# BenChung/SuccessiveConvexification

Measured on AMD Instinct MI355X. Metric: 6-DoF K=50 SCvx iterations/sec (batch), higher is better.
Workload: dtype f64

## Files before the change

successiveconvexification_amd/csrc/scvx_ipm_core.hpp:

```cpp
#pragma once
#include <math.h>
#include <stdint.h>
#include <type_traits>

#if defined(__HIPCC__)
#define SCVX_HD __host__ __device__ __forceinline__
#define SCVX_HD_NI __host__ __device__ __attribute__((noinline))
#else
#define SCVX_HD inline
#define SCVX_HD_NI inline
#endif
#if defined(SCVX_IPM_PROF) && defined(__HIP_DEVICE_COMPILE__)
#define SCVX_TS(v) const unsigned long long v = __builtin_amdgcn_s_memtime()
#define SCVX_TE(v, slot) prof[slot] += (double)(__builtin_amdgcn_s_memtime() - v)
#else
#define SCVX_TS(v)
#define SCVX_TE(v, slot)
#endif
#ifndef SCVX_NODE_QR
#define SCVX_NODE_QR 0
#endif
#ifndef SCVX_STALL_ITERS
#define SCVX_STALL_ITERS 3
#endif
#ifndef SCVX_INIT_BALANCE
#define SCVX_INIT_BALANCE 1.0
#endif
#ifndef SCVX_INIT_SHIFT
#define SCVX_INIT_SHIFT 0.25
#endif
#ifndef SCVX_WARM_RADIUS
#define SCVX_WARM_RADIUS 0.999
#endif
#ifndef SCVX_BLEND_WARM
#define SCVX_BLEND_WARM 0.0
#endif
#ifndef SCVX_BLEND_RADIUS
#define SCVX_BLEND_RADIUS 0.9
#endif
#ifndef SCVX_STEP_FRAC
#define SCVX_STEP_FRAC 0.98
#endif
#ifndef SCVX_REFINE_PRED
#define SCVX_REFINE_PRED 0
#endif
#ifndef SCVX_BLOWUP_STOP
#define SCVX_BLOWUP_STOP 10.0
#endif
#ifndef SCVX_WARM_SAVE
#define SCVX_WARM_SAVE 1.0
#endif
#ifndef SCVX_FACTOR_T
#define SCVX_FACTOR_T double
#endif
#ifndef SCVX_STREAM_U
#define SCVX_STREAM_U 4
#endif
#ifndef SCVX_REFINE_FROM
#define SCVX_REFINE_FROM 1e-4
#endif
#ifndef SCVX_REFINE_FUSED
#define SCVX_REFINE_FUSED 1
#endif
#ifndef SCVX_FUSED_RES
#define SCVX_FUSED_RES 0
#endif
#ifndef SCVX_NEWTON_CORR_ATTR
#define SCVX_NEWTON_CORR_ATTR SCVX_HD
#endif
#ifndef SCVX_CARRY_BIGSUMS
#define SCVX_CARRY_BIGSUMS 0
#endif
#ifndef SCVX_RESID_UPDATE
#define SCVX_RESID_UPDATE 1
#endif
#ifndef SCVX_RESID_FRESH_FROM
#define SCVX_RESID_FRESH_FROM 1e-4
#endif
#ifndef SCVX_TWISTED_TSPACE
#define SCVX_TWISTED_TSPACE 1
#endif
#ifndef SCVX_REFINE_STOP
#define SCVX_REFINE_STOP 0.1
#endif
#if defined(__HIPCC__)
#define SCVX_UNROLL _Pragma("unroll")
#else
#define SCVX_UNROLL
#endif
#if defined(__HIP_DEVICE_COMPILE__) && !defined(SCVX_NO_LDS_FRAME)
#define SCVX_THIS_LDS() do { __builtin_assume(__builtin_amdgcn_is_shared((const void*)this)); __builtin_assume(__builtin_amdgcn_is_shared((const void*)&C)); } while (0)
#else
#define SCVX_THIS_LDS() do { } while (0)
#endif
#define SCVX_T0() SCVX_TS(t0_)
#define SCVX_T1(slot) SCVX_TE(t0_, slot)
#if defined(SCVX_IPM_DEBUG) && !defined(__HIPCC__)
#include <stdio.h>
#ifndef SCVX_DBG_NODE
#define SCVX_DBG_NODE -1
#endif
#define SCVX_DBG(...) fprintf(stderr, __VA_ARGS__)
#else
#define SCVX_DBG(...)
#endif

#if defined(SCVX_COUNTERS) && !defined(__HIPCC__)
extern "C" long long scvx_counters[8];
#define SCVX_COUNT(i) do { _Pragma("omp atomic") scvx_counters[i]++; } while (0)
#else
#define SCVX_COUNT(i)
#endif

namespace scvx {
namespace ipm {

#if defined(__HIP_DEVICE_COMPILE__)
#define SCVX_GLOBAL __attribute__((address_space(1)))
#else
#define SCVX_GLOBAL
#endif
template <class T> struct gp {
    typedef SCVX_GLOBAL T elem;
    typedef elem* ptr;
    typedef const elem* cptr;
};
typedef gp<double>::elem gdouble;
typedef gp<double>::ptr gptr;
typedef gp<double>::cptr cgptr;

struct Consts {
    int K, max_iter, refine, pad;
    int warm, retries;
    double tol, accept;
    double itan, sqcm, icos, Tmax, Tmin, omMax, mdry, wNu, mwet;
    double finmxf;
    double vmax;
    double rIf[3], vIf[3], qBIf[4], wBi[3], wBf[3];
};

enum { LINV_SZ = 105 };
SCVX_HD int linv_row(int i) { return i < 7 ? 15 * i : 15 * (13 - i) + (14 - i); }

enum { HX_M = 0, HX_R = 1, HX_V = 10, HX_Q = 19, HX_Q34 = 20, HX_W = 24, HX_SZ = 33 };
SCVX_HD constexpr int hu_size(int nu) { return nu == 5 ? 13 : 9; }

struct Layout {
    int K, nx, nu_, nloc, nv, iS, iTNU, iTTR, iTS;
    int o_gs, o_tilt, o_rate, o_mass, o_tb, o_tc, o_lb, o_fin, o_dp, o_nu, o_tr, o_sg, o_rk, nc;
    int c_gs, c_tilt, c_rate, c_mass, c_tb, c_tc, c_lb, c_fin, c_dp, c_nu, c_tr, c_sg, c_rk, ncones, nsmall;
    int ndp, nfin, NU;
    int ny;
    SCVX_HD void init(int K_, bool with_dp = false, int nu = 3) {
        K = K_;
        NU = nu == 5 ? 5 : 3;
        ndp = with_dp ? K_ : 0;
        nfin = NU == 5 ? K_ + 1 : 0;
        nx = 14 * (K + 1);
        nu_ = NU * (K + 1);
        nloc = nx + nu_ + 14 * K;
        iS = nloc; iTNU = nloc + 1; iTTR = nloc + 2; iTS = nloc + 3;
        nv = nloc + 4;
        ny = 14 * K;
        o_gs = 0; o_tilt = 3 * K; o_rate = 6 * K; o_mass = 10 * K; o_tb = 11 * K;
        o_tc = o_tb + 4 * (K + 1); o_lb = o_tc + 4 * (K + 1); o_fin = o_lb + (K + 1); o_dp = o_fin + 3 * nfin; o_nu = o_dp + 4 * ndp;
        o_tr = o_nu + 14 * K + 1; o_sg = o_tr + (14 + NU) * (K + 1) + 1; o_rk = o_sg + 2; nc = o_rk + 1;
        c_gs = 0; c_tilt = K; c_rate = 2 * K; c_mass = 3 * K; c_tb = 4 * K; c_tc = c_tb + K + 1; c_lb = c_tc + K + 1;
        c_fin = c_lb + K + 1;
        c_dp = c_fin + nfin;
        nsmall = c_dp + ndp;
        c_nu = nsmall; c_tr = nsmall + 1; c_sg = nsmall + 2; c_rk = nsmall + 3; ncones = nsmall + 4;
    }
    SCVX_HD size_t work_doubles() const {
        size_t n = 0;
        n += (size_t)ny;
        n += (size_t)nv * 8;
        n += (size_t)ny * 10;
        n += (size_t)nc * 8;
        n += (size_t)ncones;
        n += (size_t)(K + 1) * HX_SZ + (size_t)(K + 1) * hu_size(NU);
        n += (size_t)K * (LINV_SZ + 196);
        n += (size_t)K * 196;
        n += (size_t)ny;
        n += (size_t)ny * 4 + nloc;
        n += (size_t)nloc * 2;
        n += (size_t)3 * (K + 1);
        n += (size_t)(K + 1);
        n += 64;
        n += (size_t)nv + ny + 2 * (size_t)nc + 8;
        return n;
    }
};

template <class PS, class PZ, class PV>
SCVX_HD void soc_nt_small(PS s, PZ z, int d, PV v, double& beta) {
    double s1 = 0, z1 = 0, sz = 0;
    for (int i = 1; i < d; i++) { s1 += s[i] * s[i]; z1 += z[i] * z[i]; sz += s[i] * z[i]; }
    const double sj = sqrt(s[0] * s[0] - s1), zj = sqrt(z[0] * z[0] - z1);
    const double isj = 1.0 / sj, izj = 1.0 / zj;
    const double gam = sqrt(0.5 * (1.0 + (s[0] * z[0] + sz) * isj * izj));
    const double ig = 0.5 / gam;
    const double wb0 = (s[0] * isj + z[0] * izj) * ig;
    const double den = 1.0 / sqrt(2.0 * (wb0 + 1.0));
    v[0] = (wb0 + 1.0) * den;
    for (int i = 1; i < d; i++) v[i] = (s[i] * isj - z[i] * izj) * ig * den;
    beta = sqrt(sj * izj);
}
template <class PV, class PX, class PY>
SCVX_HD void soc_W_small(PV v, double beta, int d, PX x, PY y, bool inverse) {
    double vx = v[0] * x[0];
    if (!inverse) { for (int i = 1; i < d; i++) vx += v[i] * x[i]; }
    else { for (int i = 1; i < d; i++) vx -= v[i] * x[i]; }
    const double sc = inverse ? 1.0 / beta : beta;
    const double y0 = (2.0 * vx * v[0] - x[0]) * sc;
    for (int i = 1; i < d; i++) y[i] = ((inverse ? -2.0 : 2.0) * vx * v[i] + x[i]) * sc;
    y[0] = y0;
}
SCVX_HD void soc_w2(const double v0, const double n1, const double beta, double& h00, double& h01, double& h11, double& b2) {
    b2 = 1.0 / (beta * beta);
    const double a = 2.0 * v0 * v0 - 1.0;
    h00 = b2 * (a * a + 4.0 * v0 * v0 * n1);
    h01 = b2 * (-4.0 * v0 * (v0 * v0 + n1));
    h11 = b2 * 8.0 * v0 * v0;
}
SCVX_HD double soc_maxstep_parts(double l0, double d0, double ll, double ld, double dd) {
    double amax = INFINITY;
    if (d0 < 0.0) amax = -l0 / d0;
    const double a = dd, b = 2.0 * ld, c = ll;
    const double disc = b * b - 4.0 * a * c;
    if (disc >= 0.0) {
        const double sq = sqrt(disc);
        const double qq = -0.5 * (b + (b >= 0.0 ? sq : -sq));
        const double r1 = (qq != 0.0) ? c / qq : INFINITY;
        const double r2 = (a != 0.0) ? qq / a : INFINITY;
        if (r1 > 0.0 && r1 < amax) amax = r1;
        if (r2 > 0.0 && r2 < amax) amax = r2;
    }
    return amax;
}
SCVX_HD double piv_floor(double p, double diag) { const double f = 1e-15 * diag; return p > f ? p : f; }
template <class PO>
SCVX_HD void inv3(const double* M, PO Mi) {
    const double l00 = sqrt(M[0]);
    const double l10 = M[3] / l00, l20 = M[6] / l00;
    const double l11 = sqrt(piv_floor(M[4] - l10 * l10, M[4]));
    const double l21 = (M[7] - l20 * l10) / l11;
    const double l22 = sqrt(piv_floor(M[8] - l20 * l20 - l21 * l21, M[8]));
    const double i00 = 1.0 / l00, i11 = 1.0 / l11, i22 = 1.0 / l22;
    const double i10 = -l10 * i00 * i11;
    const double i21 = -l21 * i11 * i22;
    const double i20 = -(l20 * i00 + l21 * i10) * i22;
    Mi[0] = i00 * i00 + i10 * i10 + i20 * i20;
    Mi[1] = Mi[3] = i10 * i11 + i20 * i21;
    Mi[2] = Mi[6] = i20 * i22;
    Mi[4] = i11 * i11 + i21 * i21;
    Mi[5] = Mi[7] = i21 * i22;
    Mi[8] = i22 * i22;
}
template <class PO>
SCVX_HD void inv2(double a, double b, double d, PO Mi) {
    const double l00 = sqrt(a), l10 = b / l00, l11 = sqrt(piv_floor(d - l10 * l10, d));
    const double i00 = 1.0 / l00, i11 = 1.0 / l11, i10 = -l10 * i00 * i11;
    Mi[0] = i00 * i00 + i10 * i10; Mi[1] = Mi[2] = i10 * i11; Mi[3] = i11 * i11;
}

template <class PO>
SCVX_HD void inv_iso_rank1_3(double a, double kappa, double v0, double v1, double v2, PO Mi) {
    const double n2 = v0 * v0 + v1 * v1 + v2 * v2;
    const double den = 1.0 / (a + kappa * n2), ia = 1.0 / a;
    const double off = -kappa * ia * den;
    Mi[0] = (a + kappa * (v1 * v1 + v2 * v2)) * ia * den;
    Mi[4] = (a + kappa * (v0 * v0 + v2 * v2)) * ia * den;
    Mi[8] = (a + kappa * (v0 * v0 + v1 * v1)) * ia * den;
    Mi[1] = Mi[3] = off * v0 * v1;
    Mi[2] = Mi[6] = off * v0 * v2;
    Mi[5] = Mi[7] = off * v1 * v2;
}
template <class PO>
SCVX_HD void inv_iso_rank1_2(double a, double kappa, double v0, double v1, PO Mi) {
    const double den = 1.0 / (a + kappa * (v0 * v0 + v1 * v1)), ia = 1.0 / a;
    Mi[0] = (a + kappa * v1 * v1) * ia * den;
    Mi[3] = (a + kappa * v0 * v0) * ia * den;
    Mi[1] = Mi[2] = -kappa * v0 * v1 * ia * den;
}
template <int D>
SCVX_HD void soc_Winv_col(const double* v, double ibeta, const double* x, double* y) {
    double vx = v[0] * x[0];
    for (int i = 1; i < D; i++) vx -= v[i] * x[i];
    y[0] = (2.0 * vx * v[0] - x[0]) * ibeta;
    for (int i = 1; i < D; i++) y[i] = (-2.0 * vx * v[i] + x[i]) * ibeta;
}
template <int NR, class PO>
SCVX_HD void qr_inv3(double (&A)[NR][3], PO Mi) {
    double R[3][3] = {{0, 0, 0}, {0, 0, 0}, {0, 0, 0}};
    for (int j = 0; j < 3; j++) {
// ... 854 lines not shown
                       const double vn = w.e + alpha * w.f;
                       s[i] = sn; z[i] = zn; vnb[i] = vn;
                       const double rn = sn - vn;
                       q0 += sn * sn; q1 += zn * zn; q2 += sn * zn; q3 += sn * rn; q4 += zn * rn; q5 += rn * rn;
                   });
            bigs[q][0] = ex.sum(q0); bigs[q][1] = ex.sum(q1); bigs[q][2] = ex.sum(q2);
            bigs[q][3] = ex.sum(q3); bigs[q][4] = ex.sum(q4); bigs[q][5] = ex.sum(q5);
            if (ex.lane() == 0) {
                s[0] = s0 + alpha * (d0 - (s0 - a0));
                z[0] = z0 + alpha * ((2.0 * vx * v0 - b0) * ibeta);
            }
        }
        ex.sync();
        for (int i = L.nloc + ex.lane(); i < L.nv; i += ex.nlanes()) Vn[i] = V_[i] + alpha * dw_[i];
        bigs_ok = true;
        {
            const gptr y_ = y; const cgptr dy_ = dy;
            stream(0, L.ny, [&](int i) { return D2{y_[i], dy_[i]}; }, [&](int i, const D2& v) { y_[i] = v.a + alpha * v.b; });
        }
        ex.sync();
        SCVX_T1(23);
    }

    SCVX_HD_NI void Hb_inv(cgptr g, gptr out, bool with_nu = true) {
        SCVX_THIS_LDS();
        SCVX_T0();
        const int K = L.K;
        const cgptr hx_ = hx; const cgptr hu_ = hu;
        stream(0, L.nx,
               [&](int t) {
                   const int k = t / 14, j = t - 14 * k;
                   const int hb = j == 0 ? HX_M : j < 4 ? HX_R + 3 * (j - 1) : j < 7 ? HX_V + 3 * (j - 4) : j < 9 ? HX_Q
                                  : j < 11 ? HX_Q34 + 2 * (j - 9) : HX_W + 3 * (j - 11);
                   const int gb = j == 0 ? 0 : j < 4 ? 1 : j < 7 ? 4 : j < 9 ? j : j < 11 ? 9 : 11;
                   const int n = (j == 0 || j == 7 || j == 8) ? 1 : (j == 9 || j == 10) ? 2 : 3;
                   cgptr h = hx_ + (size_t)k * HX_SZ + hb; cgptr x = g + 14 * k + gb;
                   const int i1 = n > 1 ? 1 : 0, i2 = n > 2 ? 2 : 0;
                   return D6{h[0], n > 1 ? h[i1] : 0.0, n > 2 ? h[i2] : 0.0, x[0], x[i1], x[i2]};
               },
               [&](int t, const D6& w) { out[t] = w.a * w.d + w.b * w.e + w.c * w.f; });
        {
            cgptr gu = g + L.nx; gptr ou = out + L.nx;
            stream(0, L.nu_,
                   [&](int t) {
                       const int k = t / NU, c = t - NU * k;
                       if (NU == 3 || c < 3) { cgptr h = hu_ + HU_SZ * k + 3 * c; cgptr x = gu + NU * k; return D6{h[0], h[1], h[2], x[0], x[1], x[2]}; }
                       cgptr h = hu_ + HU_SZ * k + 9 + 2 * (c - 3); cgptr x = gu + NU * k + 3;
                       return D6{h[0], h[1], 0.0, x[0], x[1], 0.0};
                   },
                   [&](int t, const D6& w) { ou[t] = w.a * w.d + w.b * w.e + w.c * w.f; });
        }
        if (with_nu) {
            cgptr gn = g + L.nx + L.nu_; gptr on = out + L.nx + L.nu_;
            const double hn = hnui;
            stream<8>(0, 14 * K, [&](int i) { return gn[i]; }, [&](int i, double v) { on[i] = hn * v; });
        }
        ex.sync();
        SCVX_T1(3);
    }

    SCVX_HD bool twisted() const { return Ex::kTwisted && L.K >= 8; }
    template <int N>
    SCVX_HD void chains_fwd(const cgptr (&tz)[N], const gptr (&x)[N]) {
        const int K = L.K;
        const cfptr Nf = this->Nf;
        if constexpr (Ex::kTwisted) {
            if (twisted()) {
                const int m = K / 2;
                ex.template chain_range_n<N>(0, K, tz, Nf, x, false, 0, m, true);
                ex.template chain_range_n<N>(2, K, tz, Nf, x, true, K - 1, K - 1 - m, true);
                ex.sync();
                for (int e = ex.lane(); e < 14 * N; e += ex.nlanes()) {
                    const int q = e / 14, i = e - 14 * q;
                    cfptr Na = Nf + (size_t)m * 196 + i;
                    cfptr Nb = Nf + (size_t)(m + 1) * 196 + 14 * i;
                    cgptr xa = x[q] + 14 * (m - 1); cgptr xb = x[q] + 14 * (m + 1);
                    double a = tz[q][14 * m + i];
                    for (int j = 0; j < 14; j++) a += Na[14 * j] * xa[j] + Nb[j] * xb[j];
                    x[q][14 * m + i] = a;
                }
                ex.sync();
                return;
            }
        }
        ex.template chain_n<N>(K, tz, Nf, x, false);
        ex.sync();
    }
    template <int N>
    SCVX_HD void chains_bwd(const cgptr (&xz)[N], const gptr (&t)[N]) {
        const int K = L.K;
        const cfptr Nf = this->Nf;
        if constexpr (Ex::kTwisted) {
            if (twisted()) {
                const int m = K / 2;
                ex.template chain_range_n<N>(0, K, xz, Nf, t, true, m, m + 1, true);
                ex.template chain_range_n<N>(2, K, xz, Nf, t, false, m, K - m, false);
                ex.sync();
                return;
            }
        }
        ex.template chain_n<N>(K, xz, Nf, t, true);
        ex.sync();
    }
    template <int N>
    SCVX_HD void solve_chains(const gptr (&t)[N], const gptr (&x)[N]) {
        cgptr tz[N], xz[N];
        for (int q = 0; q < N; q++) { tz[q] = t[q]; xz[q] = x[q]; }
        chains_fwd<N>(tz, x);
        chains_bwd<N>(xz, t);
    }
    SCVX_HD_NI void S_solve(cgptr r, gptr x) {
        SCVX_THIS_LDS();
        SCVX_T0();
        const int K = L.K;
        const cfptr Linv = this->Linv;
        const gptr tchain = this->tchain;
        for (int t = ex.lane(); t < 14 * K; t += ex.nlanes()) {
            const int k = t / 14, i = t - 14 * k;
            cfptr Li = Linv + (size_t)k * LINV_SZ + linv_row(i);
            cgptr rk_ = r + 14 * k;
            double a = 0;
#if defined(__HIPCC__)
#pragma unroll
#endif
            for (int j = 0; j < 14; j++) a += (j <= i ? Li[j <= i ? j : i] : 0.0) * rk_[j];
            tchain[t] = a;
        }
        ex.sync();
        SCVX_TE(t0_, 16);
        SCVX_TS(tc1_);
        {
            const gptr ts[1] = {tchain};
            const gptr xs[1] = {x};
            solve_chains<1>(ts, xs);
        }
        SCVX_TE(tc1_, 17);
        SCVX_TS(tp2_);
        for (int t = ex.lane(); t < 14 * K; t += ex.nlanes()) {
            const int k = t / 14, i = t - 14 * k;
            cfptr Lk = Linv + (size_t)k * LINV_SZ;
            cgptr wk = tchain + 14 * k;
            double a = 0;
#if defined(__HIPCC__)
#pragma unroll
#endif
            for (int j = 0; j < 14; j++) a += (j >= i ? Lk[linv_row(j) + (j >= i ? i : j)] : 0.0) * wk[j];
            x[t] = a;
        }
        ex.sync();
        SCVX_TE(tp2_, 18);
        SCVX_T1(0);
    }

    SCVX_HD_NI void S_fwd(cgptr r, gptr t) {
        SCVX_THIS_LDS();
        SCVX_T0();
        const int K = L.K;
        const cfptr Linv = this->Linv;
        const gptr tchain = this->tchain;
        for (int e = ex.lane(); e < 14 * K; e += ex.nlanes()) {
            const int k = e / 14, i = e - 14 * k;
            cfptr Li = Linv + (size_t)k * LINV_SZ + linv_row(i);
            cgptr rk_ = r + 14 * k;
            double a = 0;
            SCVX_UNROLL
            for (int j = 0; j < 14; j++) a += (j <= i ? Li[j <= i ? j : i] : 0.0) * rk_[j];
            tchain[e] = a;
        }
        ex.sync();
        SCVX_TE(t0_, 16);
        SCVX_TS(tc1_);
        {
            const cgptr tz[1] = {tchain};
            const gptr xs[1] = {t};
            chains_fwd<1>(tz, xs);
        }
        SCVX_TE(tc1_, 17);
        SCVX_T1(0);
    }

    template <int N>
    SCVX_HD_NI void S_solveN(const cgptr (&r)[N], const gptr (&x)[N], const gptr (&t)[N]) {
        SCVX_THIS_LDS();
        const int K = L.K;
        const cfptr Linv = this->Linv;
        for (int e = ex.lane(); e < 14 * K; e += ex.nlanes()) {
            const int k = e / 14, i = e - 14 * k;
            cfptr Li = Linv + (size_t)k * LINV_SZ + linv_row(i);
            double a[N];
            for (int q = 0; q < N; q++) a[q] = 0;
            SCVX_UNROLL
            for (int j = 0; j < 14; j++) {
                const double l = j <= i ? Li[j <= i ? j : i] : 0.0;
                for (int q = 0; q < N; q++) a[q] += l * r[q][14 * k + j];
            }
            for (int q = 0; q < N; q++) t[q][e] = a[q];
        }
        ex.sync();
        solve_chains<N>(t, x);
        for (int e = ex.lane(); e < 14 * K; e += ex.nlanes()) {
            const int k = e / 14, i = e - 14 * k;
            cfptr Lk = Linv + (size_t)k * LINV_SZ;
            double a[N];
            for (int q = 0; q < N; q++) a[q] = 0;
            SCVX_UNROLL
            for (int j = 0; j < 14; j++) {
                const double l = j >= i ? Lk[linv_row(j) + (j >= i ? i : j)] : 0.0;
                for (int q = 0; q < N; q++) a[q] += l * t[q][14 * k + j];
            }
            for (int q = 0; q < N; q++) x[q][e] = a[q];
        }
        ex.sync();
    }
    template <int N>
    SCVX_HD_NI void S_backN(const gptr (&x)[N], const gptr (&t)[N]) {
        SCVX_THIS_LDS();
        const int K = L.K;
        const cfptr Linv = this->Linv;
        cgptr xz[N];
        for (int q = 0; q < N; q++) xz[q] = x[q];
        chains_bwd<N>(xz, t);
        for (int e = ex.lane(); e < 14 * K; e += ex.nlanes()) {
            const int k = e / 14, i = e - 14 * k;
            cfptr Lk = Linv + (size_t)k * LINV_SZ;
            double a[N];
            for (int q = 0; q < N; q++) a[q] = 0;
            SCVX_UNROLL
            for (int j = 0; j < 14; j++) {
                const double l = j >= i ? Lk[linv_row(j) + (j >= i ? i : j)] : 0.0;
                for (int q = 0; q < N; q++) a[q] += l * t[q][14 * k + j];
            }
            for (int q = 0; q < N; q++) x[q][e] = a[q];
        }
        ex.sync();
    }
    SCVX_HD_NI void E_apply2(cgptr v0, cgptr v1, gptr out0, gptr out1, cgptr add1) {
        SCVX_THIS_LDS();
        SCVX_T0();
        const int K = L.K;
        for (int r = ex.lane(); r < 14 * K; r += ex.nlanes()) {
            const int k = r / 14, i = r - 14 * k;
            dcptr Dk = D + (size_t)k * DSZ + i;
            const double ad = add1[r];
            double a = 0, b = 0;
            for (int j = 0; j < 14; j++) { const double d = Dk[14 * j]; a += d * v0[14 * k + j]; b += d * v1[14 * k + j]; }
            for (int j = 0; j < 2 * NU; j++) { const double d = Dk[14 * (14 + j)]; a += d * v0[L.nx + NU * k + j]; b += d * v1[L.nx + NU * k + j]; }
            a += v0[L.nx + L.nu_ + r] - v0[14 * (k + 1) + i];
            b += v1[L.nx + L.nu_ + r] - v1[14 * (k + 1) + i];
            out0[r] = a;
            out1[r] = b + ad;
        }
        ex.sync();
        SCVX_T1(1);
    }

    template <class E2 = Ex>
    SCVX_HD_NI bool factor_pipelined(bool with_pred) {
        SCVX_THIS_LDS();
        const int K = L.K;
        const dcptr D_ = D; const cgptr hx_ = hx; const cgptr hu_ = hu;
        const fptr Linv_ = Linv; const fptr Nf_ = Nf;
        const double hnui_ = hnui;
        double* sc = ex.pipe_scratch();
        double* Sd = sc;
        double* So = Sd + 392;
        double* Wp = So + 392;
        double* Li = Wp + 588;
        double* Mq = Li + 392;
        double* Dt = Mq + 392;
        double* T = Dt + DSZ;
        double* Bp = T + 14 * TS;
        double* Hh = Bp + BPN;
        double* Hd = Hh + 2 * NODE_SZ;
        double* Gn = Hd + 196;
        double* Rr = Gn + 2 * NXU * 4;
        double* Tt = Rr + 168;
        double* Sg = Tt + 112;
        const int w = ex.wave(), l = ex.wlane();
        bool ok = true;
        auto node_elem = [&](int node, int e) -> double {
            return e < HX_SZ ? hx_[(size_t)node * HX_SZ + e] : hu_[HU_SZ * node + (e - HX_SZ)];
        };
        const cgptr Wtr_ = Wv + L.o_tr + 1; const cgptr Wnu_ = Wv + L.o_nu + 1; const cgptr gx_ = gx; const cgptr ry_ = ry;
        const int nx_ = L.nx, nxu_ = L.nx + L.nu_;
        auto gnode_elem = [&](int nd, int e) -> double {
            const int vec = e >= NXU ? 1 : 0, row = e - NXU * vec;
            if (vec == 1 && !with_pred) return 0.0;
            cgptr src = vec ? gx_ : Wtr_;
            return row < 14 ? src[14 * nd + row] : src[nx_ + NU * nd + (row - 14)];
        };
        auto gseg_elem = [&](int sgk, int e) -> double {
            if (e >= 28) return Wnu_[14 * sgk + (e - 28)];
            if (!with_pred) return 0.0;
            return e < 14 ? gx_[nxu_ + 14 * sgk + e] : ry_[14 * sgk + (e - 14)];
        };
        const gptr xq_[4] = {ys, ytr, ynu, dy};
        if (w == 1) {
            for (int e = l; e < 2 * NXU * 4; e += 64) Gn[e] = 0.0;
            ex.w_sync_lds();
            for (int e = l; e < 2 * NXU; e += 64) {
                const int vec = e >= NXU ? 1 : 0, row = e - NXU * vec;
                Gn[NXU * 4 + 4 * row + (vec ? 3 : 1)] = gnode_elem(0, e);
            }
            for (int e = l; e < DSZ; e += 64) Dt[e] = D_[e];
            for (int e = l; e < NODE_SZ; e += 64) Hh[NODE_SZ + e] = node_elem(0, e);
            ex.w_sync_lds();
            for (int e = l; e < 196; e += 64) Hd[e] = hxi_entry(Hh + NODE_SZ, e / 14, e % 14);
            ex.w_sync_lds();
            ex.w_tile_gemm(T, TS, 1, Dt, 1, 14, Hd, 14, 1, 14, 1.0, false);
            for (int q = l; q < BPN; q += 64) {
                const int i = q / NU, c = q - NU * i;
                T[TS * i + 14 + c] = bhu(Dt, 14, i, c, Hh + NODE_SZ + HX_SZ);
            }
            ex.w_sync_lds();
        }
        const int hpos_lane = hx_dense_pos(l <= HX_SZ ? l : 0);
        typename E2::WAcc cg;
        ex.w_acc_zero(cg);
        double gnacc = 0.0;
        double hnext = (w == 1 && l < NODE_SZ) ? node_elem(1, l) : 0.0;
        double gnext = (w == 1 && l < 2 * NXU) ? gnode_elem(1, l) : 0.0;
        double sgnext = (w == 1 && l < 42) ? gseg_elem(0, l) : 0.0;
        auto fwd_subst = [&](int kp) {
// ... 1214 lines not shown
                }
                ex.sync_lds();
                SCVX_TE(te_, 26);
                SCVX_TS(te2_);
                ex.tile_gemm(T, TS, 1, Dt, 1, 14, Hd, 14, 1, 14, 1.0, false);
                for (int q = ex.lane(); q < BPN; q += ex.nlanes()) {
                    const int i = q / NU, c = q - NU * i;
                    T[TS * i + 14 + c] = bhu(Dt, 14, i, c, Hh + NODE_SZ + HX_SZ);
                }
                ex.sync_lds();
                SCVX_TE(te2_, 27);
                SCVX_TS(te3_);
                for (int e = ex.lane(); e < 196; e += ex.nlanes()) {
                    const int i = e / 14, j = e - 14 * i;
                    M[e] = so_elem(T, Bp, i, j);
                }
                ex.sync_lds();
                SCVX_TE(te3_, 28);
                SCVX_TS(te4_);
                ex.tile_gemm(Wp, 14, 1, M, 14, 1, Li, 1, 14, 14, 1.0, false);
                SCVX_TE(te4_, 29);
            }
            SCVX_TS(te5_);
            if (res) {
                const bool lastn = k + 1 == K;
                for (int row = ex.lane(); row < NXU; row += ex.nlanes()) {
                    double ev = 0.0;
                    if (!lastn) {
                        for (int i = 0; i < 14; i++) ev += Dt[14 * row + i] * Yv[14 + i];
                        if (row < 14) ev -= Yv[row];
                        else for (int i = 0; i < 14; i++) ev += Bp[14 * (row - 14) + i] * Yv[i];
                    } else {
                        if (row < 14) ev = -Yv[row];
                        else for (int i = 0; i < 14; i++) ev += Dt[14 * (NU + row) + i] * Yv[i];
                    }
                    const bool fx = lastn && (row < 14 ? fixed_x(K, row) : fixed_u(K, row - 14));
                    const double rxv = fx ? 0.0 : Pn[NXU + row] + ev;
                    const double gxv = fx ? 0.0 : Gn[NXU * 4 + 4 * row + 3] - ev;
                    Gn[NXU * 4 + 4 * row + 3] = gxv;
                    const int at = row < 14 ? 14 * (k + 1) + row : nx_ + NU * (k + 1) + (row - 14);
                    rx_[at] = rxv; gx_[at] = gxv;
                    nrx2 += rxv * rxv;
                }
            }
            ex.sync_lds();
            {
                typename Ex::Acc cr;
                ex.acc_zero(cr);
                ex.acc_mac(cr, T + 14 + NU, TS, 1, Gn + NXU * 4 + 14 * 4, 4, 1, NU, 1.0, 4);
                ex.acc_mac(cr, Hd, 14, 1, Gn + NXU * 4, 4, 1, 14, -1.0, 4);
                ex.acc_store(cr, Rk, 4, 1, true, 4);
            }
            ex.sync_lds();
            for (int i = ex.lane(); i < 14; i += ex.nlanes()) {
                Rk[4 * i] = Sk[i];
                Rk[4 * i + 2] = hnui_ * Sg[28 + i];
                Rk[4 * i + 3] += hnui_ * Sg[i] + Sg[14 + i];
                gnacc += Sg[28 + i] * Sg[i];
            }
            ex.sync_lds();
            SCVX_TE(te5_, 30);
            SCVX_TS(te6_);
            ex.acc_mac(ct, Li, 14, 1, Rk, 4, 1, 14, 1.0, 4);
            ex.acc_store(ct, Tc, 4, 1, false, 4);
            ex.sync_lds();
            ex.acc_mac(cg, Tc, 1, 4, Tc, 4, 1, 14, 1.0, 4);
            for (int e = ex.lane(); e < 56; e += ex.nlanes()) {
                const int q = e / 14, i = e - 14 * q;
                if (q < 3 || with_pred) xq_[q][14 * k + i] = Tc[4 * i + q];
            }
            SCVX_TE(te6_, 31);
        }
        if (res) { res_nrx2 = ex.sum(nrx2); res_nry2 = ex.sum(nry2); res_sgy = ex.sum(sgacc); }
        ex.sync_lds();
        ex.acc_store(cg, Rk, 4, 1, false, 4);
        ex.sync_lds();
        for (int q = 0; q < 16; q++) gram[q] = Rk[q];
        gn_pred = ex.sum(gnacc);
        }
        ex.sync();
        SCVX_TE(tC_, 6);
        SCVX_TS(tB_);
        tsp = kFusedBorder;
        if (kFusedBorder) {
            Hb_inv(Wv + L.o_tr + 1, ptl, false);
            const double ptp = dot(Wv + L.o_tr + 1, ptl, L.nx + L.nu_);
            css = gram[0]; cst = -gram[1]; csn = -gram[2];
            cts = -gram[1]; ctt = -ptp + gram[5]; ctn = gram[6];
            cns = -gram[2]; cnt_ = gram[6]; pny = gram[10] / hnui_;
            SCVX_TE(tB_, 7);
            return ex.all(ok);
        } else {
            const int nxu = L.nx + L.nu_;
            const gptr g_tr = r1;
            {
                cgptr wt = Wv + L.o_tr + 1;
                stream<8>(0, L.nloc, [&](int i) { return i < nxu ? wt[i] : 0.0; }, [&](int i, double v) { g_tr[i] = v; });
            }
            ex.sync();
            Hb_inv(g_tr, ptl);
            if (with_pred) {
                Hb_inv(gx, cw);
                E_apply2(ptl, cw, rtr, rp, ry);
            } else {
                E_apply(ptl, rtr, false);
            }
            {
                gptr ty = tmpy; gptr r2_ = r2; cgptr wn = Wv + L.o_nu + 1;
                stream(0, L.ny, [&](int r) { const int k = r / 14, i = r - 14 * k; return D2{D_[(size_t)k * DSZ + 14 * CS + i], wn[r]}; },
                       [&](int r, const D2& v) { ty[r] = v.a; r2_[r] = hnui_ * v.b; });
            }
            ex.sync();
            if (with_pred) {
                const cgptr rr[4] = {tmpy, rtr, r2, rp};
                const gptr xx[4] = {ys, ytr, ynu, dy};
                const gptr tt4[4] = {tchain, cy, tq0, tq1};
                S_solveN<4>(rr, xx, tt4);
            } else {
                const cgptr rr[3] = {tmpy, rtr, r2};
                const gptr xx[3] = {ys, ytr, ynu};
                const gptr tt3[3] = {tchain, cy, tq0};
                S_solveN<3>(rr, xx, tt3);
            }
        }
        {
            double a[9];
            for (int q = 0; q < 9; q++) a[q] = 0.0;
            {
                cgptr y0 = ys; cgptr y1 = ytr; cgptr y2 = ynu; cgptr rt = rtr; cgptr wn = Wv + L.o_nu + 1;
                stream(0, L.ny, [&](int r) { const int k = r / 14, i = r - 14 * k; return D6{D_[(size_t)k * DSZ + 14 * CS + i], y0[r], y1[r], y2[r], rt[r], wn[r]}; },
                       [&](int, const D6& v) {
                           a[0] += v.a * v.b; a[1] += v.a * v.c; a[2] += v.a * v.d;
                           a[3] += v.e * v.b; a[4] += v.e * v.c; a[5] += v.e * v.d;
                           a[6] += v.f * v.b; a[7] += v.f * v.c; a[8] += v.f * v.d;
                       });
            }
            for (int q = 0; q < 9; q++) a[q] = ex.sum(a[q]);
            const double ptp = dot(Wv + L.o_tr + 1, ptl, L.nx + L.nu_);
            css = a[0]; cst = -a[1]; csn = -a[2];
            cts = -a[3]; ctt = -ptp + a[4]; ctn = a[5];
            cns = -hnui_ * a[6]; cnt_ = hnui_ * a[7]; pny = a[8];
        }
        SCVX_TE(tB_, 7);
        return ex.all(ok);
    }

    SCVX_HD void kkt_solve(cgptr g, cgptr ryv, gptr dwv, gptr dyv, double rsign = 1.0, bool have_band = false, gptr eout = nullptr,
                           double* sgout = nullptr) {
        double c0s, c0t, c0n;
        if (tsp) {
            double a0, a1, a2, gn;
            if (have_band) { a0 = gram[3]; a1 = gram[7]; a2 = gram[11]; gn = gn_pred; }
            else {
                Hb_inv(g, tmpl);
                (void)E_apply(tmpl, tmpy, false, ryv, -rsign);
                S_fwd(tmpy, dyv);
                double q0 = 0, q1 = 0, q2 = 0, q3 = 0;
                cgptr b0 = ys; cgptr b1 = ytr; cgptr b2 = ynu; cgptr wn = Wv + L.o_nu + 1; cgptr gnu = g + L.nx + L.nu_;
                stream(0, L.ny, [&](int i) { return D6{dyv[i], b0[i], b1[i], b2[i], wn[i], gnu[i]}; },
                       [&](int, const D6& v) { q0 += v.a * v.b; q1 += v.a * v.c; q2 += v.a * v.d; q3 += v.e * v.f; });
                a0 = ex.sum(q0); a1 = ex.sum(q1); a2 = ex.sum(q2); gn = ex.sum(q3);
            }
            c0s = a0;
            c0t = dot(ptl, g, L.nx + L.nu_) - a1;
            c0n = hnui * gn - a2;
        } else {
        if (!have_band) {
            Hb_inv(g, tmpl);
            (void)E_apply(tmpl, tmpy, false, ryv, -rsign);
            S_solve(tmpy, dyv);
        }
        double a = 0, bt = 0, bn = 0, gn = 0;
        {
            const dcptr D_ = D; cgptr rt = rtr; cgptr wn = Wv + L.o_nu + 1; cgptr gnu = g + L.nx + L.nu_;
            stream(0, L.ny, [&](int r) { const int k = r / 14, i = r - 14 * k; return D5{D_[(size_t)k * DSZ + 14 * CS + i], dyv[r], rt[r], wn[r], gnu[r]}; },
                   [&](int, const D5& v) { a += v.a * v.b; bt += v.c * v.b; bn += v.d * v.b; gn += v.d * v.e; });
        }
        c0s = ex.sum(a);
        bt = ex.sum(bt); bn = ex.sum(bn); gn = ex.sum(gn);
        c0t = dot(ptl, g, L.nx + L.nu_) - bt;
        c0n = hnui * (gn - bn);
        }
        const double v0n = q_nu[0], n1n = q_nu[1], h00n = h_nu[0], h01n = h_nu[1];
        const double v0t = q_tr[0], b2t = h_tr[3], h01t = h_tr[1];
        const double dtt = h_tr[0] + hrk;
        const double sig_t = 8.0 * v0t * v0t * b2t * (hrk - b2t) / dtt, kap_t = h01t * g[L.iTTR] / dtt;
        const double sig_n = -8.0 * v0n * v0n / (hnui * hnui * h00n), kap_n = h01n * g[L.iTNU] / h00n;
        const double v0s = q_sg[0], vs = q_sg[1];
        double M[9], r[3];
        M[0] = q_sg[2] / (1.0 + 8.0 * v0s * v0s * vs * vs) + css; M[1] = cst; M[2] = csn;
        r[0] = g[L.iS] - c0s - q_sg[3] * g[L.iTS];
        M[3] = -sig_t * cts; M[4] = 1.0 - sig_t * ctt; M[5] = -sig_t * ctn; r[1] = kap_t + sig_t * c0t;
        M[6] = cns; M[7] = cnt_; M[8] = hnui * (pny + 1.0 / (8.0 * v0n * v0n));
        r[2] = -c0n - (v0n * v0n + n1n) * g[L.iTNU] * hnui / (2.0 * v0n);
        for (int c = 0; c < 3; c++) {
            int p = c; double best = fabs(M[c * 3 + c]);
            for (int i = c + 1; i < 3; i++) if (fabs(M[i * 3 + c]) > best) { best = fabs(M[i * 3 + c]); p = i; }
            if (p != c) { for (int j = 0; j < 3; j++) { const double t = M[c * 3 + j]; M[c * 3 + j] = M[p * 3 + j]; M[p * 3 + j] = t; } const double t = r[c]; r[c] = r[p]; r[p] = t; }
            const double ip = 1.0 / M[c * 3 + c];
            for (int i = c + 1; i < 3; i++) {
                const double f = M[i * 3 + c] * ip;
                for (int j = c; j < 3; j++) M[i * 3 + j] -= f * M[c * 3 + j];
                r[i] -= f * r[c];
            }
        }
        double b[3];
        for (int i = 2; i >= 0; i--) { double a_ = r[i]; for (int j = i + 1; j < 3; j++) a_ -= M[i * 3 + j] * b[j]; b[i] = a_ / M[i * 3 + i]; }
        const double s_ = b[0], ctr = b[1], cnu = b[2];
        const double pi_t = c0t + cts * s_ + ctt * ctr + ctn * cnu;
        const double pi_n = (cnu - kap_n) / sig_n;
        const double ttr_ = (g[L.iTTR] - h01t * pi_t) / dtt;
        const double tnu_ = (g[L.iTNU] - h01n * pi_n) / h00n;
        const double ts_ = g[L.iTS] / h00s - q_sg[3] * s_;
        ex.sync();
        {
            cgptr b0 = ys; cgptr b1 = ytr; cgptr b2 = ynu;
            stream(0, L.ny, [&](int i) { return D4{dyv[i], b0[i], b1[i], b2[i]}; },
                   [&](int i, const D4& v) { dyv[i] = v.a + v.b * s_ - v.c * ctr - v.d * cnu; });
        }
        ex.sync();
        if (tsp) {
            const gptr xx[1] = {dyv};
            const gptr tt[1] = {tchain};
            S_backN<1>(xx, tt);
        }
        {
            const double sg_ = Et_apply(dyv, tmpl2, g, 1, ctr, cnu, eout);
            if (sgout) *sgout = sg_;
        }
        Hb_inv(tmpl2, dwv);
        if (ex.lane() == 0) { dwv[L.iS] = s_; dwv[L.iTS] = ts_; dwv[L.iTNU] = tnu_; dwv[L.iTTR] = ttr_; }
        ex.sync();
    }

    SCVX_HD_NI void H_apply(cgptr dwv, gptr out) {
        SCVX_THIS_LDS();
        cone_map(dwv, tmpc, false);
        ex.sync();
        W_all(tmpc, tmpc, true);
        W_all(tmpc, tmpc, true);
        cone_map_t(tmpc, out);
        ex.sync();
    }

    SCVX_HD void newton_solve(bool pred) {
        if (!pred) {
            cone_map_t(tmpc, gx, rx);
            mask_fixed(gx);
        }
        SCVX_COUNT(0);
        kkt_solve(gx, ry, dw, dy, -1.0, pred);
#if defined(SCVX_IPM_DEBUG) && !defined(__HIPCC__)
        {
            H_apply(dw, r1);
            const double sgy = Et_apply(dy, tmpl);
            double e1 = 0, e2 = 0, e3 = 0;
            for (int i = 0; i < L.nloc; i++) { double r = gx[i] - r1[i] - tmpl[i]; bool fx = false;
                if (i < 14) fx = fixed_x(0, i); else if (i >= 14 * L.K && i < L.nx) fx = fixed_x(L.K, i - 14 * L.K); else if (i == L.nx + NU * L.K + 1 || i == L.nx + NU * L.K + 2) fx = true;
                if (!fx) { if (i < L.nx + L.nu_) e1 += r * r; else e2 += r * r; } }
            E_apply(dw, tmpy2, true);
            for (int i = 0; i < L.ny; i++) { double r = -ry[i] - tmpy2[i]; e3 += r * r; }
            SCVX_DBG("      kkt res: xu %.2e nu %.2e s %.2e tnu %.2e ttr %.2e ts %.2e | E %.2e\n", sqrt(e1), sqrt(e2), gx[L.iS] - r1[L.iS] - sgy,
                     gx[L.iTNU] - r1[L.iTNU], gx[L.iTTR] - r1[L.iTTR], gx[L.iTS] - r1[L.iTS], sqrt(e3));
        }
#endif
        const int nref = (cur_gate < SCVX_REFINE_FROM && !(pred && !SCVX_REFINE_PRED)) ? C.refine : 0;
        double nr_prev = INFINITY;
        for (int it = 0; it < nref; it++) {
            SCVX_COUNT(1);
            H_apply(dw, r1);
            const double sgy = Et_apply(dy, tmpl);
            ex.sync();
            {
                gptr r1_ = r1; cgptr g_ = gx; cgptr tl = tmpl;
                stream(0, L.nloc, [&](int i) { return D3{g_[i], r1_[i], tl[i]}; }, [&](int i, const D3& v) { r1_[i] = v.a - v.b - v.c; });
            }
            ex.sync();
            if (ex.lane() == 0) {
                r1[L.iS] = gx[L.iS] - r1[L.iS] - sgy;
                r1[L.iTNU] = gx[L.iTNU] - r1[L.iTNU];
                r1[L.iTTR] = gx[L.iTTR] - r1[L.iTTR];
                r1[L.iTS] = gx[L.iTS] - r1[L.iTS];
            }
            ex.sync();
            mask_fixed(r1);
            const double nr1 = sqrt(sumsq(r1, L.nv));
            SCVX_DBG("      refine %d: |r1| %.3e\n", it, nr1);
#if defined(SCVX_IPM_DEBUG) && !defined(__HIPCC__)
            if (it == 0) {
                int am = 0; double mx = 0;
                for (int i = 0; i < L.nv; i++) if (fabs((double)r1[i]) > mx) { mx = fabs((double)r1[i]); am = i; }
                if (am < L.nx) SCVX_DBG("        max at x node %d comp %d (%.3e)\n", am / 14, am % 14, mx);
                else if (am < L.nx + L.nu_) SCVX_DBG("        max at u node %d comp %d (%.3e)\n", (am - L.nx) / NU, (am - L.nx) % NU, mx);
                else SCVX_DBG("        max at index %d of nv %d (%.3e)\n", am, L.nv, mx);
            }
#endif
            if (nr1 <= SCVX_REFINE_STOP * C.tol * (C.wNu > 1.0 ? C.wNu : 1.0)) break;
            if (it > 0 && !(nr1 < 0.5 * nr_prev)) break;
            nr_prev = nr1;
            E_apply(dw, tmpy2, true);
            ex.sync();
            {
                gptr t2 = tmpy2; cgptr ry_ = ry;
                stream(0, L.ny, [&](int i) { return D2{ry_[i], t2[i]}; }, [&](int i, const D2& v) { t2[i] = -v.a - v.b; });
            }
            ex.sync();
            SCVX_COUNT(2);
            kkt_solve(r1, tmpy2, cw, cy);
            {
// ... 369 lines not shown
```

Before: 145,900.

## Fuse Hb_inv, E_apply and S_fwd into a single pipelined front sweep

Replaces the three passes Hb_inv, E_apply and the first Cholesky-inverse product in S_fwd with one sweep over time steps. Per-step H-scaled gradient blocks sit in a small LDS ring, and the loads for the next chunk are software-prefetched into registers while the current chunk is computed. The aim is to drop the intermediate global round-trips through tmpl and tmpy and the full-block syncs between passes. In exchange it adds more LDS barriers per chunk, needs more registers for the prefetched D rows, and uses __dmul_rn to keep rounding consistent.

```diff
diff --git a/successiveconvexification_amd/csrc/scvx_ipm_core.hpp b/successiveconvexification_amd/csrc/scvx_ipm_core.hpp
--- a/successiveconvexification_amd/csrc/scvx_ipm_core.hpp
+++ b/successiveconvexification_amd/csrc/scvx_ipm_core.hpp
@@ -141,6 +141,14 @@
 
 enum { LINV_SZ = 105 };
 SCVX_HD int linv_row(int i) { return i < 7 ? 15 * i : 15 * (13 - i) + (14 - i); }
+
+SCVX_HD double mul_rn(double a, double b) {
+#if defined(__HIP_DEVICE_COMPILE__)
+    return __dmul_rn(a, b);
+#else
+    return a * b;
+#endif
+}
 
 enum { HX_M = 0, HX_R = 1, HX_V = 10, HX_Q = 19, HX_Q34 = 20, HX_W = 24, HX_SZ = 33 };
 SCVX_HD constexpr int hu_size(int nu) { return nu == 5 ? 13 : 9; }
@@ -1301,23 +1309,117 @@
         SCVX_T1(0);
     }
 
-    SCVX_HD_NI void S_fwd(cgptr r, gptr t) {
+    static constexpr int SW_CH = Ex::kLanes >= 14 ? Ex::kLanes / 14 : 4;
+    static constexpr int SW_NS = SW_CH + 1;
+    static constexpr bool SW_ONE = Ex::kLanes >= 14 * SW_CH;
+    SCVX_HD double* sweep_lds() {
+        if constexpr (Ex::kPipelineFactor) return ex.pipe_scratch(); else return ex.scratch() + 32;
+    }
+    struct SwA { D6 hx, hu; };
+    struct SwB { double d[14 + 2 * NU], ad, gv; };
+    struct SwC { double l[14]; };
+    SCVX_HD D6 sw_hx_row(cgptr g, int k, int j) const {
+        const int hb = j == 0 ? HX_M : j < 4 ? HX_R + 3 * (j - 1) : j < 7 ? HX_V + 3 * (j - 4) : j < 9 ? HX_Q
+                       : j < 11 ? HX_Q34 + 2 * (j - 9) : HX_W + 3 * (j - 11);
+        const int gb = j == 0 ? 0 : j < 4 ? 1 : j < 7 ? 4 : j < 9 ? j : j < 11 ? 9 : 11;
+        const int n = (j == 0 || j == 7 || j == 8) ? 1 : (j == 9 || j == 10) ? 2 : 3;
+        cgptr h = hx + (size_t)k * HX_SZ + hb; cgptr x = g + 14 * k + gb;
+        const int i1 = n > 1 ? 1 : 0, i2 = n > 2 ? 2 : 0;
+        return D6{h[0], n > 1 ? h[i1] : 0.0, n > 2 ? h[i2] : 0.0, x[0], x[i1], x[i2]};
+    }
+    SCVX_HD D6 sw_hu_row(cgptr g, int k, int c) const {
+        cgptr gu = g + L.nx;
+        if (NU == 3 || c < 3) { cgptr h = hu + HU_SZ * k + 3 * c; cgptr x = gu + NU * k; return D6{h[0], h[1], h[2], x[0], x[1], x[2]}; }
+        cgptr h = hu + HU_SZ * k + 9 + 2 * (c - 3); cgptr x = gu + NU * k + 3;
+        return D6{h[0], h[1], 0.0, x[0], x[1], 0.0};
+    }
+    SCVX_HD void sw_load_b(SwB& w, cgptr g, cgptr add, int k, int i) const {
+        dcptr Dk = D + (size_t)k * DSZ + i;
+        SCVX_UNROLL
+        for (int j = 0; j < 14 + 2 * NU; j++) w.d[j] = Dk[14 * j];
+        w.ad = add[14 * k + i];
+        w.gv = g[L.nx + L.nu_ + 14 * k + i];
+    }
+    SCVX_HD void sw_load_c(SwC& w, int k, int i) const {
+        cfptr Li = Linv + (size_t)k * LINV_SZ + linv_row(i);
+        SCVX_UNROLL
+        for (int j = 0; j < 14; j++) w.l[j] = j <= i ? (double)Li[j <= i ? j : i] : 0.0;
+    }
+    static SCVX_HD double sw_hb(const D6& w) { return w.a * w.d + w.b * w.e + w.c * w.f; }
+    SCVX_HD double sw_erow(const SwB& w, const double* Hs, int k, int i, double hn, double sa) const {
+        const double* hk = Hs + NXU * (k % SW_NS); const double* hk1 = Hs + NXU * ((k + 1) % SW_NS);
+        double a = 0;
+        SCVX_UNROLL
+        for (int j = 0; j < 14 + NU; j++) a += w.d[j] * hk[j];
+        SCVX_UNROLL
+        for (int j = 0; j < NU; j++) a += w.d[14 + NU + j] * hk1[14 + j];
+        a += mul_rn(hn, w.gv) - hk1[i];
+        a += sa * w.ad;
+        return a;
+    }
+    static SCVX_HD double sw_lrow(const SwC& w, const double* rk_) {
+        double a = 0;
+        SCVX_UNROLL
+        for (int j = 0; j < 14; j++) a += w.l[j] * rk_[j];
+        return a;
+    }
+    SCVX_HD_NI void front_sweep(cgptr g, cgptr add, double sa, gptr t) {
         SCVX_THIS_LDS();
         SCVX_T0();
-        const int K = L.K;
-        const cfptr Linv = this->Linv;
-        const gptr tchain = this->tchain;
-        for (int e = ex.lane(); e < 14 * K; e += ex.nlanes()) {
-            const int k = e / 14, i = e - 14 * k;
-            cfptr Li = Linv + (size_t)k * LINV_SZ + linv_row(i);
-            cgptr rk_ = r + 14 * k;
-            double a = 0;
-            SCVX_UNROLL
-            for (int j = 0; j < 14; j++) a += (j <= i ? Li[j <= i ? j : i] : 0.0) * rk_[j];
-            tchain[e] = a;
-        }
-        ex.sync();
-        SCVX_TE(t0_, 16);
+        const int K = L.K, nl = ex.nlanes(), ln = ex.lane();
+        const double hn = hnui;
+        const gptr tchain_ = tchain;
+        double* Hs = sweep_lds();
+        double* Rs = Hs + SW_NS * NXU;
+        for (int e = ln; e < NXU; e += nl) Hs[e] = sw_hb(e < 14 ? sw_hx_row(g, 0, e) : sw_hu_row(g, 0, e - 14));
+        if constexpr (SW_ONE) {
+            auto load_ab = [&](SwA& a, SwB& b, int k0) {
+                const int ns = K - k0 < SW_CH ? K - k0 : SW_CH;
+                const int e = ln < 14 * ns ? ln : 0, eu = ln < NU * ns ? ln : 0;
+                a.hx = sw_hx_row(g, k0 + 1 + e / 14, e % 14);
+                a.hu = sw_hu_row(g, k0 + 1 + eu / NU, eu % NU);
+                sw_load_b(b, g, add, k0 + e / 14, e % 14);
+            };
+            SwA a; SwB b;
+            load_ab(a, b, 0);
+            for (int k0 = 0; k0 < K; k0 += SW_CH) {
+                const int ns = K - k0 < SW_CH ? K - k0 : SW_CH;
+                const bool on = ln < 14 * ns;
+                const int kk = on ? ln / 14 : 0, i = on ? ln - 14 * kk : 0, k = k0 + kk;
+                SwC c;
+                sw_load_c(c, k, i);
+                if (on) Hs[NXU * ((k + 1) % SW_NS) + i] = sw_hb(a.hx);
+                if (ln < NU * ns) Hs[NXU * ((k0 + 1 + ln / NU) % SW_NS) + 14 + ln % NU] = sw_hb(a.hu);
+                SwA an = a; SwB bn = b;
+                if (k0 + SW_CH < K) load_ab(an, bn, k0 + SW_CH);
+                ex.sync_lds();
+                if (on) Rs[ln] = sw_erow(b, Hs, k, i, hn, sa);
+                ex.sync_lds();
+                if (on) tchain_[14 * k + i] = sw_lrow(c, Rs + 14 * kk);
+                a = an; b = bn;
+            }
+        } else {
+            for (int k0 = 0; k0 < K; k0 += SW_CH) {
+                const int ns = K - k0 < SW_CH ? K - k0 : SW_CH;
+                for (int e = ln; e < 14 * ns; e += nl) Hs[NXU * ((k0 + 1 + e / 14) % SW_NS) + e % 14] = sw_hb(sw_hx_row(g, k0 + 1 + e / 14, e % 14));
+                for (int e = ln; e < NU * ns; e += nl) Hs[NXU * ((k0 + 1 + e / NU) % SW_NS) + 14 + e % NU] = sw_hb(sw_hu_row(g, k0 + 1 + e / NU, e % NU));
+                ex.sync_lds();
+                for (int e = ln; e < 14 * ns; e += nl) {
+                    SwB w;
+                    sw_load_b(w, g, add, k0 + e / 14, e % 14);
+                    Rs[e] = sw_erow(w, Hs, k0 + e / 14, e % 14, hn, sa);
+                }
+                ex.sync_lds();
+                for (int e = ln; e < 14 * ns; e += nl) {
+                    SwC w;
+                    sw_load_c(w, k0 + e / 14, e % 14);
+                    tchain_[14 * (k0 + e / 14) + e % 14] = sw_lrow(w, Rs + 14 * (e / 14));
+                }
+                ex.sync_lds();
+            }
+        }
+        ex.sync();
+        SCVX_TE(t0_, 14);
         SCVX_TS(tc1_);
         {
             const cgptr tz[1] = {tchain};
@@ -2838,9 +2940,7 @@
             double a0, a1, a2, gn;
             if (have_band) { a0 = gram[3]; a1 = gram[7]; a2 = gram[11]; gn = gn_pred; }
             else {
-                Hb_inv(g, tmpl);
-                (void)E_apply(tmpl, tmpy, false, ryv, -rsign);
-                S_fwd(tmpy, dyv);
+                front_sweep(g, ryv, -rsign, dyv);
                 double q0 = 0, q1 = 0, q2 = 0, q3 = 0;
                 cgptr b0 = ys; cgptr b1 = ytr; cgptr b2 = ynu; cgptr wn = Wv + L.o_nu + 1; cgptr gnu = g + L.nx + L.nu_;
                 stream(0, L.ny, [&](int i) { return D6{dyv[i], b0[i], b1[i], b2[i], wn[i], gnu[i]}; },
```

Measured after the change: 147,700, median of 6. +1.3%, better.
